# alanqrwang/nwhead

Hardware: AMD Instinct MI355X
Metric: query-predictions/sec (higher is better)
Workload: dtype f32; 1 GPU; K3 predict('full'): B=256 queries/step vs bank N=50000 d=512 C=200, bank sharded 1-way, 26 query batches coalesced per launch; B=256, N_support=50000, d=512, C=200, parallelism=support-shard x1

## Files before the change

nwhead_amd/csrc/fused_f16p.h:

```cpp
#pragma once
#include "fused_impl.h"
#include "persistent_pipe.h"

namespace nw {
namespace {

template <int RS, int QB, bool TWO = false>
struct PCfg : PipeCfg<16 * RS, 64 * QB, NCONS, NLOAD, TWO ? 3 : 4> {};

template <int RS, int KIND, int QB, int NCW = NCONS>
__device__ __forceinline__ void epilogue_p(f32x4 (&acc)[QB][RS], const float* hdr, int nrun, int2 bnd,
                                           const float* __restrict__ logit_scale, float* __restrict__ ws_m,
                                           float* __restrict__ ws_den, float* __restrict__ ws_num, int B, int N,
                                           int q0, int s0, int st, int wave, int lane
#ifdef NW_DIAG_FUSED
                                           , unsigned long long (&diag_)[8], unsigned long long& last_
#endif
                                           ) {
    using P = PCfg<RS, QB>;
    constexpr int BS = P::BS;
    constexpr bool NEED_NORM = (KIND != NW_SCORE_DOT);
    constexpr float L2E = 1.44269504088896340736f;
    typedef float f32x2 __attribute__((ext_vector_type(2)));
    const float* sn2 = hdr;
// ... 83 lines not shown
                    S1[r & 1] = __builtin_fmaf(in1 ? 1.f : 0.f, quad, S1[r & 1]);
                    S2[r & 1] = __builtin_fmaf(in2 ? 1.f : 0.f, quad, S2[r & 1]);
                    if (!(in0 || in1 || in2)) {
#pragma unroll
                        for (int e = 0; e < 4; ++e) {
                            const float c = (float)(16 * r + e), ev = sc[r][e];
                            const float w1 = __builtin_amdgcn_fmed3f(L1 - c, 0.f, 1.f);
                            const float u2 = __builtin_amdgcn_fmed3f(c + M2, 0.f, 1.f);
                            S0[e & 1] = __builtin_fmaf(w1, ev, S0[e & 1]);
                            S2[e & 1] = __builtin_fmaf(u2, ev, S2[e & 1]);
                            S1[e & 1] = __builtin_fmaf((1.f - w1) - u2, ev, S1[e & 1]);
                        }
                    }
                }
            }
            const float s0v = red4(S0[0] + S0[1]);
            float s1v = 0.f, s2v = 0.f;
            if (nrun >= 2) s1v = red4(S1[0] + S1[1]);
            if (nrun == 3) s2v = red4(S2[0] + S2[1]);
            dloc = (s0v + s1v) + s2v;
            if (g == 0 && b < B) {
                ws_num[((size_t)st * BS) * B + b] = s0v;
                if (nrun >= 2) ws_num[((size_t)st * BS + 1) * B + b] = s1v;
                if (nrun == 3) ws_num[((size_t)st * BS + 2) * B + b] = s2v;
            }
        } else {
            float dl[4] = {0.f, 0.f, 0.f, 0.f};
#pragma unroll
            for (int r = 0; r < RS; ++r) dl[r & 3] += (sc[r][0] + sc[r][1]) + (sc[r][2] + sc[r][3]);
            dloc = red4((dl[0] + dl[1]) + (dl[2] + dl[3]));
            for (int run_base = 0; run_base < nrun; run_base += 16) {
                f32x4 Pm = {0.f, 0.f, 0.f, 0.f};
                const int want = run_base + i;
#pragma unroll
                for (int r = 0; r < RS; ++r) {
                    const int4 rid = *reinterpret_cast<const int4*>(runid + 16 * r + 4 * g);
                    Pm = __builtin_amdgcn_mfma_f32_16x16x4f32(rid.x == want ? 1.f : 0.f, sc[r][0], Pm, 0, 0, 0);
                    Pm = __builtin_amdgcn_mfma_f32_16x16x4f32(rid.y == want ? 1.f : 0.f, sc[r][1], Pm, 0, 0, 0);
                    Pm = __builtin_amdgcn_mfma_f32_16x16x4f32(rid.z == want ? 1.f : 0.f, sc[r][2], Pm, 0, 0, 0);
                    Pm = __builtin_amdgcn_mfma_f32_16x16x4f32(rid.w == want ? 1.f : 0.f, sc[r][3], Pm, 0, 0, 0);
                }
                if (b < B) {
#pragma unroll
                    for (int jj = 0; jj < 4; ++jj) {
                        const int run = run_base + 4 * g + jj;
                        if (run < nrun) ws_num[((size_t)st * BS + run) * B + b] = Pm[jj];
                    }
                }
            }
        }
        NW_PSTAMP(4);
        if (g == 0 && b < B) {
            ws_m[(size_t)st * B + b] = mloc;
            ws_den[(size_t)st * B + b] = dloc;
        }
        NW_PSTAMP(5);
    }
}

template <int RS, int KIND, bool TWO, int QB>
__global__ __launch_bounds__(TILE_THREADS, TWO ? 4 : 2) void nw_fused_f16p_kernel(
    const float* __restrict__ q, const float* __restrict__ s, const float* __restrict__ s_norm2,
    const float* __restrict__ s_scale, const float* __restrict__ q_norm2, const float* __restrict__ q_scale,
    const float* __restrict__ logit_scale, const int* __restrict__ ws_runid, const int* __restrict__ ws_nrun, const int* __restrict__ ws_bnd,
    float* __restrict__ ws_m, float* __restrict__ ws_den, float* __restrict__ ws_num, int B, int N, int d,
    int n_stiles, int n_qtiles, int qg) {
    using P = PCfg<RS, QB, TWO>;
    constexpr int BS = P::BS, BQP = P::BQP, TILE_F4 = P::TILE_F4, NB = P::NB;
    constexpr bool SINGLE = TWO || QB > 1;
    static_assert(!(TWO && QB > 1), "two 128-query workgroups do not fit the LDS of a CU");
    static_assert(P::THREADS == TILE_THREADS, "launch bounds");
    static_assert(RS == 8, "the persistent kernel is built for tiles of 128 supports");
    extern __shared__ __attribute__((aligned(16))) char smem[];
    float* hdr0 = reinterpret_cast<float*>(smem);
    float4* stage = reinterpret_cast<float4*>(smem + P::HDR_BYTES);

    const int tid = threadIdx.x, lane = tid & 63;
    const int wave = __builtin_amdgcn_readfirstlane(tid >> 6);
    const int nk = d / BK;
    const PersistentTiles tiles(blockIdx.x, gridDim.x, n_stiles, n_qtiles, qg);
    const int cu = tiles.cu, n_cu = tiles.n_cu, n_local = tiles.n_local;

    if (wave >= P::NCW) {
        persistent_loader<P>(tiles, wave - P::NCW, lane, hdr0, stage, q, s, s_norm2, s_scale, q_norm2, q_scale, ws_runid, B, N,
                             d);
    } else {
        const int i = lane & 15, g = lane >> 4;
        struct Frag {
            float4 bh[QB], bl[QB];
            float4 ah[RS], al[RS];
        };
        const int rsw = (i >> 1) & 7;
        auto load_frags = [&](Frag& f, int buf) {
            const float4* Qs = stage + ((unsigned)buf % NB) * TILE_F4;
            const float4* Ss = Qs + BQP * ROW_F4;
            const int sh = g ^ rsw, sl = (4 + g) ^ rsw;
#pragma unroll
            for (int j = 0; j < QB; ++j) {
                const int qrow = 16 * (QB * wave + j) + i;
                f.bh[j] = Qs[qrow * ROW_F4 + sh];
                f.bl[j] = Qs[qrow * ROW_F4 + sl];
            }
#pragma unroll
            for (int r = 0; r < RS; ++r) {
                f.ah[r] = Ss[(16 * r + i) * ROW_F4 + sh];
                f.al[r] = Ss[(16 * r + i) * ROW_F4 + sl];
            }
        };
        auto mm = [](const float4& a, const float4& b, f32x4 c) {
            return __builtin_amdgcn_mfma_f32_16x16x32_f16(__builtin_bit_cast(half8, a), __builtin_bit_cast(half8, b), c, 0, 0, 0);
        };
        f32x4 acc[QB][RS];
        auto mfma_stage = [&](const Frag& f) {
#pragma unroll
            for (int j = 0; j < QB; ++j)
#pragma unroll
                for (int r = 0; r < RS; ++r) acc[j][r] = mm(f.al[r], f.bh[j], acc[j][r]);
#pragma unroll
            for (int j = 0; j < QB; ++j)
#pragma unroll
                for (int r = 0; r < RS; ++r) acc[j][r] = mm(f.ah[r], f.bl[j], acc[j][r]);
#pragma unroll
            for (int j = 0; j < QB; ++j)
#pragma unroll
                for (int r = 0; r < RS; ++r) acc[j][r] = mm(f.ah[r], f.bh[j], acc[j][r]);
        };
        auto interleave = [&]() {
#pragma unroll
            for (int x = 0; x < 2 * (RS + 1); ++x) {
                __builtin_amdgcn_sched_group_barrier(0x008, 1, 0);
                __builtin_amdgcn_sched_group_barrier(0x100, 1, 0);
            }
            __builtin_amdgcn_sched_group_barrier(0x008, 3 * RS - 2 * (RS + 1), 0);
        };

        tile_barrier();
        int gi = 0;
        int par = 0;
#ifdef NW_DIAG_FUSED
        unsigned long long diag_[8] = {0, 0, 0, 0, 0, 0, 0, 0}, last_ = __builtin_amdgcn_s_memtime();
        const unsigned long long first_ = last_, first_rt_ = __builtin_amdgcn_s_memrealtime();
#endif
        for (int T = cu; T < n_local; T += n_cu) {
            int qt, st;
            tiles.decode(T, qt, st);
            const int q0 = qt * BQP, s0 = st * BS;
            const int nrun = ws_nrun[st];
            const int2 bnd = *reinterpret_cast<const int2*>(ws_bnd + 2 * (size_t)st);

#pragma unroll
            for (int j = 0; j < QB; ++j)
#pragma unroll
                for (int r = 0; r < RS; ++r) acc[j][r] = f32x4{0.f, 0.f, 0.f, 0.f};
            if constexpr (QB > 1) {
                struct F1 { float4 bh[QB]; float4 al[RS]; };
                struct F2 { float4 bl[QB]; float4 ah[RS]; };
                const int sh = g ^ rsw, sl = (4 + g) ^ rsw;
                const int qoff = (16 * QB * wave + i) * ROW_F4, soff = (BQP + i) * ROW_F4;
                auto stage_base = [&](int buf) { return stage + ((unsigned)buf % NB) * TILE_F4; };
                auto rd_bh = [&](const float4* S, int j) { return S[qoff + 16 * j * ROW_F4 + sh]; };
                auto rd_bl = [&](const float4* S, int j) { return S[qoff + 16 * j * ROW_F4 + sl]; };
                auto rd_ah = [&](const float4* S, int r) { return S[soff + 16 * r * ROW_F4 + sh]; };
                auto rd_al = [&](const float4* S, int r) { return S[soff + 16 * r * ROW_F4 + sl]; };
                auto pin = []() { __builtin_amdgcn_sched_barrier(0); };
                auto run_stage = [&](const F1& ac, F1& an, F2& b, int buf_next, auto has_next) {
#ifdef NW_ABL_NORD
                    constexpr bool NXT = false;
// ... 128 lines not shown
```

nwhead_amd/csrc/fused_f16p12.h:

```cpp
#pragma once
#include "fused_f16p.h"

namespace nw {
namespace {

struct P12 : PipeCfg<128, 256, 8, 4, 3> {
    static constexpr int RS = BS / 16, QB = BQP / (16 * NCW);
    static_assert(LDS_BYTES <= 160 * 1024, "LDS of one CU");
};

template <int KIND, bool CAND = false>
__device__ __forceinline__ void epilogue_p12(f32x4 (&acc)[P12::QB][P12::RS], const float* hdr, int nrun, int2 bnd,
                                             float scale, float* __restrict__ ws_m,
                                             float* __restrict__ ws_den, float* __restrict__ ws_num, int B, int N,
                                             int q0, int s0, int st, int wave, int lane, int n_stiles, int k
#ifdef NW_DIAG_FUSED
                                             , unsigned long long (&diag_)[8], unsigned long long& last_
#endif
                                             ) {
    using P = P12;
    constexpr int RS = P::RS, QB = P::QB, BS = P::BS;
    constexpr bool NEED_NORM = (KIND != NW_SCORE_DOT);
    typedef float f32x2 __attribute__((ext_vector_type(2)));
    const float* sn2 = hdr;
    const float* ssc = hdr + P::NH;
    const int* runid = reinterpret_cast<const int*>(hdr + 2 * P::NH);
    const float* qn2 = hdr + 3 * P::NH;
    const float* qsc_s = qn2 + P::BQP;
    const int i = lane & 15, g = lane >> 4;
    using SF = ScoreFactors<KIND>;
    float Cq[QB], Bq[QB];
#pragma unroll
    for (int j = 0; j < QB; ++j) {
        const int qrow = 16 * (QB * wave + j) + i;
        SF::query(NEED_NORM ? qn2[qrow] : 0.f, qsc_s[qrow], scale, Cq[j], Bq[j]);
    }
    NW_PSTAMP(1);
    float sc[QB][RS][4];
#pragma unroll
    for (int r = 0; r < RS; ++r) {
        const float4 n4 = NEED_NORM ? *reinterpret_cast<const float4*>(sn2 + 16 * r + 4 * g) : make_float4(0.f, 0.f, 0.f, 0.f);
        const float4 s4 = *reinterpret_cast<const float4*>(ssc + 16 * r + 4 * g);
        float4 K4, B4;
        SF::support(n4.x, s4.x, K4.x, B4.x);
        SF::support(n4.y, s4.y, K4.y, B4.y);
        SF::support(n4.z, s4.z, K4.z, B4.z);
        SF::support(n4.w, s4.w, K4.w, B4.w);
        float4 B4r = B4;
        asm volatile("" : "+v"(B4r.x), "+v"(B4r.y), "+v"(B4r.z), "+v"(B4r.w));
#pragma unroll
        for (int j = 0; j < QB; ++j) {
            const f32x2 cq = {Cq[j], Cq[j]}, bq = {Bq[j], Bq[j]};
            const float4 Bj = (j == 0) ? B4 : B4r;
            const f32x2 d01 = __builtin_elementwise_fma(f32x2{acc[j][r][0], acc[j][r][1]}, f32x2{K4.x, K4.y} * cq,
                                                        f32x2{Bj.x, Bj.y} + bq);
            const f32x2 d23 = __builtin_elementwise_fma(f32x2{acc[j][r][2], acc[j][r][3]}, f32x2{K4.z, K4.w} * cq,
                                                        f32x2{Bj.z, Bj.w} + bq);
            sc[j][r][0] = SF::finish_abs(d01.x);
            sc[j][r][1] = SF::finish_abs(d01.y);
            sc[j][r][2] = SF::finish_abs(d23.x);
            sc[j][r][3] = SF::finish_abs(d23.y);
            asm volatile("" : "+v"(sc[j][r][0]), "+v"(sc[j][r][1]), "+v"(sc[j][r][2]), "+v"(sc[j][r][3]));
        }
        __builtin_amdgcn_sched_barrier(0);
    }
    NW_PSTAMP(2);
    if constexpr (CAND) {
        int ln = lane;
        asm volatile("" : "+v"(ln));
        const int ci = ln & 15, cg = ln >> 4;
#pragma unroll
        for (int j = 0; j < QB; ++j) {
            float u[RS][4];
#pragma unroll
            for (int r = 0; r < RS; ++r)
#pragma unroll
                for (int e = 0; e < 4; ++e) u[r][e] = SF::DIST ? -sc[j][r][e] : sc[j][r][e];
            tile_candidates<RS>(u, reinterpret_cast<unsigned*>(ws_m), reinterpret_cast<int*>(ws_den), B, N,
                                q0 + 16 * (QB * wave + j) + ci, s0, cg, st, n_stiles, k);
            __builtin_amdgcn_sched_barrier(0);
        }
        return;
    }
    constexpr float WORST = SF::DIST ? INFINITY : -INFINITY;
    if (s0 + BS > N) {
        const int lim = N - s0 - 4 * g;
#pragma unroll
        for (int j = 0; j < QB; ++j)
#pragma unroll
            for (int r = 0; r < RS; ++r)
#pragma unroll
                for (int e = 0; e < 4; ++e)
                    if (16 * r + e >= lim) sc[j][r][e] = WORST;
    }
    auto best = [](float a, float b) { return SF::DIST ? fminf(a, b) : fmaxf(a, b); };
    auto best3 = [&](float a, float b, float c) { return best(best(a, b), c); };
    static_assert(RS == 8, "chain k takes the 16-row blocks k and k + 4");
    float ext[QB];
#pragma unroll
    for (int j = 0; j < QB; ++j) {
        float mx[4];
#pragma unroll
        for (int k = 0; k < 4; ++k) mx[k] = best3(sc[j][k][0], sc[j][k][1], sc[j][k][2]);
#pragma unroll
        for (int k = 0; k < 4; ++k) mx[k] = best3(mx[k], sc[j][k][3], sc[j][k + 4][0]);
#pragma unroll
        for (int k = 0; k < 4; ++k) mx[k] = best3(mx[k], sc[j][k + 4][1], sc[j][k + 4][2]);
#pragma unroll
        for (int k = 0; k < 4; ++k) mx[k] = best(mx[k], sc[j][k + 4][3]);
        ext[j] = best(best3(mx[0], mx[1], mx[2]), mx[3]);
    }
    group4_each(ext, best);
    float mloc[QB], dloc[QB], s0v[QB], s1v[QB] = {0.f, 0.f}, s2v[QB] = {0.f, 0.f};
#pragma unroll
    for (int j = 0; j < QB; ++j) {
        mloc[j] = SF::DIST ? -ext[j] : ext[j];
#pragma unroll
        for (int r = 0; r < RS; ++r)
#pragma unroll
            for (int e = 0; e < 4; ++e)
                sc[j][r][e] = __builtin_amdgcn_exp2f(SF::DIST ? ext[j] - sc[j][r][e] : sc[j][r][e] - ext[j]);
    }
    NW_PSTAMP(3);
    auto add = [](float a, float b) { return a + b; };
    if (nrun <= 3) {
        float S0[QB][2] = {{0.f, 0.f}, {0.f, 0.f}}, S1[QB][2] = {{0.f, 0.f}, {0.f, 0.f}}, S2[QB][2] = {{0.f, 0.f}, {0.f, 0.f}};
        if (nrun == 1) {
#pragma unroll
            for (int r = 0; r < RS; ++r)
#pragma unroll
                for (int j = 0; j < QB; ++j) S0[j][r & 1] += (sc[j][r][0] + sc[j][r][1]) + (sc[j][r][2] + sc[j][r][3]);
        } else {
            const int b1 = bnd.x, b2 = (nrun == 3) ? bnd.y : BS;
            const float L1 = (float)(b1 - 4 * g);
            const float M2 = 1.f - (float)(b2 - 4 * g);
#pragma unroll
            for (int r = 0; r < RS; ++r) {
                const int lo = 16 * r, hi = 16 * r + 16;
                const bool in0 = hi <= b1, in2 = lo >= b2, in1 = lo >= b1 && hi <= b2;
#pragma unroll
                for (int j = 0; j < QB; ++j) {
                    const float quad = (sc[j][r][0] + sc[j][r][1]) + (sc[j][r][2] + sc[j][r][3]);
                    S0[j][r & 1] = __builtin_fmaf(in0 ? 1.f : 0.f, quad, S0[j][r & 1]);
                    S1[j][r & 1] = __builtin_fmaf(in1 ? 1.f : 0.f, quad, S1[j][r & 1]);
                    S2[j][r & 1] = __builtin_fmaf(in2 ? 1.f : 0.f, quad, S2[j][r & 1]);
                }
                if (!(in0 || in1 || in2)) {
#pragma unroll
                    for (int e = 0; e < 4; ++e) {
                        const float c = (float)(16 * r + e);
                        const float w1 = __builtin_amdgcn_fmed3f(L1 - c, 0.f, 1.f);
                        const float u2 = __builtin_amdgcn_fmed3f(c + M2, 0.f, 1.f);
#pragma unroll
                        for (int j = 0; j < QB; ++j) {
                            const float ev = sc[j][r][e];
                            S0[j][e & 1] = __builtin_fmaf(w1, ev, S0[j][e & 1]);
                            S2[j][e & 1] = __builtin_fmaf(u2, ev, S2[j][e & 1]);
                            S1[j][e & 1] = __builtin_fmaf((1.f - w1) - u2, ev, S1[j][e & 1]);
                        }
                    }
                }
            }
        }
        if (nrun == 1) {
            float v[QB] = {S0[0][0] + S0[0][1], S0[1][0] + S0[1][1]};
            group4_each(v, add);
            s0v[0] = v[0], s0v[1] = v[1];
        } else if (nrun == 2) {
            float v[2 * QB] = {S0[0][0] + S0[0][1], S0[1][0] + S0[1][1], S1[0][0] + S1[0][1], S1[1][0] + S1[1][1]};
            group4_each(v, add);
            s0v[0] = v[0], s0v[1] = v[1], s1v[0] = v[2], s1v[1] = v[3];
        } else {
            float v[3 * QB] = {S0[0][0] + S0[0][1], S0[1][0] + S0[1][1], S1[0][0] + S1[0][1],
                               S1[1][0] + S1[1][1], S2[0][0] + S2[0][1], S2[1][0] + S2[1][1]};
            group4_each(v, add);
            s0v[0] = v[0], s0v[1] = v[1], s1v[0] = v[2], s1v[1] = v[3], s2v[0] = v[4], s2v[1] = v[5];
        }
#pragma unroll
        for (int j = 0; j < QB; ++j) dloc[j] = (s0v[j] + s1v[j]) + s2v[j];
    } else {
#pragma unroll
        for (int j = 0; j < QB; ++j) {
            float dl[4] = {0.f, 0.f, 0.f, 0.f};
#pragma unroll
            for (int r = 0; r < RS; ++r) dl[r & 3] += (sc[j][r][0] + sc[j][r][1]) + (sc[j][r][2] + sc[j][r][3]);
            dloc[j] = (dl[0] + dl[1]) + (dl[2] + dl[3]);
        }
        group4_each(dloc, add);
#pragma unroll
        for (int j = 0; j < QB; ++j) {
            const int b = q0 + 16 * (QB * wave + j) + i;
            for (int run_base = 0; run_base < nrun; run_base += 16) {
                f32x4 Pm = {0.f, 0.f, 0.f, 0.f};
                const int want = run_base + i;
#pragma unroll
                for (int r = 0; r < RS; ++r) {
                    const int4 rid = *reinterpret_cast<const int4*>(runid + 16 * r + 4 * g);
                    Pm = __builtin_amdgcn_mfma_f32_16x16x4f32(rid.x == want ? 1.f : 0.f, sc[j][r][0], Pm, 0, 0, 0);
                    Pm = __builtin_amdgcn_mfma_f32_16x16x4f32(rid.y == want ? 1.f : 0.f, sc[j][r][1], Pm, 0, 0, 0);
                    Pm = __builtin_amdgcn_mfma_f32_16x16x4f32(rid.z == want ? 1.f : 0.f, sc[j][r][2], Pm, 0, 0, 0);
                    Pm = __builtin_amdgcn_mfma_f32_16x16x4f32(rid.w == want ? 1.f : 0.f, sc[j][r][3], Pm, 0, 0, 0);
                }
                if (b < B) {
#pragma unroll
                    for (int jj = 0; jj < 4; ++jj) {
                        const int run = run_base + 4 * g + jj;
                        if (run < nrun) ws_num[((size_t)st * BS + run) * B + b] = Pm[jj];
                    }
                }
            }
        }
    }
    NW_PSTAMP(4);
    static_assert(QB == 2, "lane groups 0 / 1 carry query blocks 0 / 1, groups 2 / 3 the same blocks of the next array");
    int ln = lane;
    asm volatile("" : "+v"(ln));
    const int b = q0 + 16 * QB * wave + (ln & 31);
    const bool blk1 = ln & 16, arr1 = ln & 32;
    const size_t tb = (size_t)st * B + b, nb = (size_t)st * BS * B + b;
    if (b < B) {
        const float mv = blk1 ? mloc[1] : mloc[0], dv = blk1 ? dloc[1] : dloc[0];
        (arr1 ? ws_den : ws_m)[tb] = arr1 ? dv : mv;
        if (nrun <= 3) {
            const float n0 = blk1 ? s0v[1] : s0v[0], n1 = blk1 ? s1v[1] : s1v[0], n2 = blk1 ? s2v[1] : s2v[0];
            if (!arr1 || nrun >= 2) ws_num[nb + (arr1 ? B : 0)] = arr1 ? n1 : n0;
            if (!arr1 && nrun == 3) ws_num[nb + 2 * (size_t)B] = n2;
        }
    }
    NW_PSTAMP(5);
}

template <int KIND, bool HALF = false, bool CAND = false>
__global__ __launch_bounds__(P12::THREADS, 3) void nw_fused_f16p_kernel_w12(
    const float* __restrict__ q, const float* __restrict__ s, const float* __restrict__ s_norm2,
    const float* __restrict__ s_scale, const float* __restrict__ q_norm2, const float* __restrict__ q_scale,
    const float* __restrict__ logit_scale, const int* __restrict__ ws_runid, const int* __restrict__ ws_nrun,
    const int* __restrict__ ws_bnd, float* __restrict__ ws_m, float* __restrict__ ws_den, float* __restrict__ ws_num, int B,
    int N, int d, int n_stiles, int n_qtiles, int qg, int k) {
    static_assert(!CAND || HALF, "the candidate form exists for half-precision rows only");
    using P = P12;
    constexpr int RS = P::RS, QB = P::QB, BS = P::BS, BQP = P::BQP, NB = P::NB;
    extern __shared__ __attribute__((aligned(16))) char smem[];
    float* hdr0 = reinterpret_cast<float*>(smem);
    float4* stage = reinterpret_cast<float4*>(smem + P::HDR_BYTES);

    const int tid = threadIdx.x, lane = tid & 63;
    const int wave = __builtin_amdgcn_readfirstlane(tid >> 6);
    const int nk = d / BK;
    const PersistentTiles tiles(blockIdx.x, gridDim.x, n_stiles, n_qtiles, qg);
    const int cu = tiles.cu, n_cu = tiles.n_cu, n_local = tiles.n_local;

    if (wave >= P::NCW) {
        persistent_loader<P, !CAND>(tiles, wave - P::NCW, lane, hdr0, stage, q, s, s_norm2, s_scale, q_norm2, q_scale, ws_runid, B, N,
                             d);
    } else {
        const int i = lane & 15, g = lane >> 4;
        const int rsw = (i >> 1) & 7;
        const int sh = g ^ rsw, sl = (4 + g) ^ rsw;
        const int qoff = (16 * QB * wave + i) * ROW_F4, soff = (BQP + i) * ROW_F4;
        struct QF { float4 bh[QB], bl[QB]; };
        struct SW { float4 al[2], ah[2]; };
        constexpr int NW_ = RS / 2;
#ifdef NW_DIAG_FUSED
        unsigned long long diag_[8] = {0, 0, 0, 0, 0, 0, 0, 0}, last_ = 0;
#endif
#ifdef NW_DIAG_HEAD
        unsigned long long h0_ = 0, h1_ = 0;
#define NW_HEAD_STAMP(t) asm volatile("s_memtime %0" : "=s"(t))
#else
#define NW_HEAD_STAMP(t)
#endif
        auto mm = [](const float4& a, const float4& b, f32x4 c) {
            return __builtin_amdgcn_mfma_f32_16x16x32_f16(__builtin_bit_cast(half8, a), __builtin_bit_cast(half8, b), c, 0, 0, 0);
        };
        auto pin = []() { __builtin_amdgcn_sched_barrier(0); };
        f32x4 acc[QB][RS];
        constexpr int NM = HALF ? 8 : 12;
        auto mm_1 = [&](const SW& w, const QF& f, int p, int m) {
            const int ph = m >> 2, x = (m >> 1) & 1, j = m & 1;
            const float4& a = HALF ? (ph == 0 ? w.ah[x] : w.al[x]) : (ph == 0 ? w.al[x] : w.ah[x]);
            const float4& b = HALF ? (ph == 0 ? f.bh[j] : f.bl[j]) : (ph == 1 ? f.bl[j] : f.bh[j]);
            acc[j][2 * p + x] = mm(a, b, acc[j][2 * p + x]);
        };
        auto mm_w = [&](const SW& w, const QF& f, int p, auto&& behind) {
#pragma unroll
            for (int m = 0; m < NM; ++m) {
                mm_1(w, f, p, m);
                behind(m);
            }
            pin();
        };
        auto nothing = [](int) {};
        typedef const __attribute__((address_space(3))) f32x4 lds_f4;
        const unsigned ring0 = (unsigned)(uintptr_t)(__attribute__((address_space(3))) char*)(char*)stage;
        unsigned a_qh = ring0 + 16u * (qoff + sh), a_ql = ring0 + 16u * (qoff + sl);
        unsigned a_sh = ring0 + 16u * (soff + sh), a_sl = ring0 + 16u * (soff + sl);
        asm volatile("" : "+v"(a_qh), "+v"(a_ql), "+v"(a_sh), "+v"(a_sl));
        auto lds_rd = [](unsigned a, int f4) { return __builtin_bit_cast(float4, *(lds_f4*)(uintptr_t)(a + 16u * f4)); };
        auto q_h = [&](int j) { return lds_rd(a_qh, 16 * j * ROW_F4); };
        auto q_l = [&](int j) { return lds_rd(a_ql, 16 * j * ROW_F4); };
        auto s_h = [&](int blk) { return lds_rd(a_sh, 16 * blk * ROW_F4); };
        auto s_l = [&](int blk) { return lds_rd(a_sl, 16 * blk * ROW_F4); };
        auto advance = [&](int slot, int m) {
            const unsigned step = (slot + 1 == NB) ? 0u - (unsigned)((NB - 1) * P::TILE_F4 * 16) : (unsigned)(P::TILE_F4 * 16);
            unsigned& a = (m == 0) ? a_qh : (m == 1) ? a_ql : (m == 2) ? a_sh : a_sl;
            a += step;
            asm volatile("" : "+v"(a));
        };
        SW wa, wb;
        auto rd_first = [&](QF& f, SW& w, int n) {
            const bool qlo = n >= 4, slo = (n < 4) != HALF;
            const int r = n & 3;
            if (r == 0 || r == 3) {
                const int x = r == 3;
                if (slo) w.al[x] = s_l(x);
                else w.ah[x] = s_h(x);
            } else {
                if (qlo) f.bl[r - 1] = q_l(r - 1);
                else f.bh[r - 1] = q_h(r - 1);
            }
        };
        auto rd_pair = [&](SW& w, int p, int n) {
            const int x = n & 1;
            if ((n < 2) != HALF) w.al[x] = s_l(2 * p + x);
            else w.ah[x] = s_h(2 * p + x);
        };
        auto run_stage = [&](const QF& fp, QF& fc, int slot, auto first) {
            constexpr bool FIRST = decltype(first)::value;
#ifdef NW_ABL_NORD
            constexpr bool RD = FIRST;
#else
            constexpr bool RD = true;
#endif
            if constexpr (FIRST) {
#pragma unroll
                for (int n = 0; n < 8; ++n) {
                    rd_first(fc, wa, n);
                    pin();
                }
            } else {
                NW_HEAD_STAMP(h0_);
                mm_w(wb, fp, NW_ - 1, [&](int m) {
                    if (m == 0) NW_HEAD_STAMP(h1_);
                    if (m < 8) {
                        pin();
                        if (RD) rd_first(fc, wa, m);
                        pin();
                    }
                });
            }
#pragma unroll
            for (int p = 0; p + 1 < NW_; ++p) {
                SW& wr = (p & 1) ? wa : wb;
                mm_w((p & 1) ? wb : wa, fc, p, [&](int m) {
                    if (m < 4) {
                        pin();
                        if (RD) rd_pair(wr, p + 1, m);
                        pin();
                    } else if (p + 2 == NW_ && m < 8) {
                        pin();
                        advance(slot, m - 4);
                        pin();
                    }
                });
            }
            static_assert(NW_ % 2 == 0, "the last pair of a stage sits in wb");
            tile_barrier();
#ifdef NW_DIAG_HEAD
            if (!FIRST) diag_[6] += h1_ - h0_;
#endif
        };
        using Yes = std::integral_constant<bool, true>;
        using No = std::integral_constant<bool, false>;

        float scale = 1.f;
        if (KIND == NW_SCORE_CLIP)
            scale = __builtin_bit_cast(float, __builtin_amdgcn_readfirstlane(__builtin_bit_cast(int, expf(*logit_scale))));
        tile_barrier();
        int gi = 0;
        int par = 0;
        auto next_slot = [&]() {
            const int b = gi;
            gi = (gi + 1 == NB) ? 0 : gi + 1;
            return b;
        };
#ifdef NW_DIAG_FUSED
        last_ = __builtin_amdgcn_s_memtime();
        const unsigned long long first_ = last_, first_rt_ = __builtin_amdgcn_s_memrealtime();
#endif
        for (int T = cu; T < n_local; T += n_cu) {
            int qt, st;
            tiles.decode(T, qt, st);
            const int q0 = qt * BQP, s0 = st * BS;
            int nrun = 0;
            int2 bnd = {0, 0};
            if constexpr (!CAND) {
                nrun = ws_nrun[st];
                bnd = *reinterpret_cast<const int2*>(ws_bnd + 2 * (size_t)st);
            }
#pragma unroll
            for (int j = 0; j < QB; ++j)
#pragma unroll
                for (int r = 0; r < RS; ++r) acc[j][r] = f32x4{0.f, 0.f, 0.f, 0.f};
            QF f0, f1;
#ifdef NW_ABL_NORD
#pragma unroll
            for (int n = 0; n < 8; ++n) rd_first(f1, wa, n);
#endif
            run_stage(f1, f0, next_slot(), Yes{});
            int kt = 1;
            for (; kt + 1 < nk; kt += 2) {
                run_stage(f0, f1, next_slot(), No{});
                run_stage(f1, f0, next_slot(), No{});
            }
            if (kt < nk) {
                run_stage(f0, f1, next_slot(), No{});
                mm_w(wb, f1, NW_ - 1, nothing);
            } else {
                mm_w(wb, f0, NW_ - 1, nothing);
            }
            NW_PSTAMP(0);
#ifndef NW_ABL_NOEPI
            epilogue_p12<KIND, CAND>(acc, hdr0 + par * P::HDR_F, nrun, bnd, scale, ws_m, ws_den, ws_num, B, N, q0, s0, st, wave,
                                     lane, n_stiles, k
#ifdef NW_DIAG_FUSED
                                     , diag_, last_
#endif
                                     );
#else
            keep_acc_alive(acc, ws_m, nrun, bnd);
#endif
            par = (par + 1 == P::NHB) ? 0 : par + 1;
#ifndef NW_DIAG_HEAD
            NW_PSTAMP(6);
#endif
        }
#ifdef NW_DIAG_FUSED
        diag_write_out(diag_, last_, first_, first_rt_);
#endif
    }
}

}
}
```

nwhead_amd/csrc/nw_internal.h:

```cpp
#pragma once
#include <hip/hip_runtime.h>
#include <stdint.h>
#include "../../include/nwhead_hip.h"

#define NW_LOG_EPS 1e-12f
#define NW_NORM_EPS 1e-12f

#define NW_CHECK_LAUNCH()                          \
    do {                                           \
        if (hipGetLastError() != hipSuccess) return NW_ERR_LAUNCH; \
    } while (0)

namespace nw {

int launch_scores(const float* q, const float* s, float* scores, int64_t B, int64_t N, int64_t d,
                  int kind, const float* logit_scale_dev, int sup_batched, hipStream_t st);

int aggregate_slices(int64_t B, int64_t N);
int launch_aggregate(const float* scores, const int64_t* sy, int labels_batched, float* out,
                     float* lse, float* weights, float* m, float* den, float* num, int64_t B,
                     int64_t N, int64_t C, hipStream_t st, float* slice_ws = nullptr, size_t slice_ws_floats = 0);

int launch_merge(const float* m, const float* den, const float* num, float* out, int64_t G,
                 int64_t B, int64_t C, int64_t sm, int64_t sd, int64_t sn, const int64_t* class_lo,
// ... 228 lines not shown
}
__device__ __forceinline__ float group4_min(float x);
__device__ __forceinline__ float group4_max(float x) {
    typedef unsigned u2_ __attribute__((ext_vector_type(2)));
    u2_ r = __builtin_amdgcn_permlane32_swap(__float_as_uint(x), __float_as_uint(x), false, false);
    x = fmaxf(__uint_as_float(r[0]), __uint_as_float(r[1]));
    r = __builtin_amdgcn_permlane16_swap(__float_as_uint(x), __float_as_uint(x), false, false);
    return fmaxf(__uint_as_float(r[0]), __uint_as_float(r[1]));
}

__device__ __forceinline__ float group4_min(float x) {
    typedef unsigned u2_ __attribute__((ext_vector_type(2)));
    u2_ r = __builtin_amdgcn_permlane32_swap(__float_as_uint(x), __float_as_uint(x), false, false);
    x = fminf(__uint_as_float(r[0]), __uint_as_float(r[1]));
    r = __builtin_amdgcn_permlane16_swap(__float_as_uint(x), __float_as_uint(x), false, false);
    return fminf(__uint_as_float(r[0]), __uint_as_float(r[1]));
}

template <int NV, typename Op>
__device__ __forceinline__ void group4_each(float (&v)[NV], Op op) {
    typedef unsigned u2_ __attribute__((ext_vector_type(2)));
    u2_ r[NV];
#pragma unroll
    for (int k = 0; k < NV; ++k) r[k] = __builtin_amdgcn_permlane32_swap(__float_as_uint(v[k]), __float_as_uint(v[k]), false, false);
#pragma unroll
    for (int k = 0; k < NV; ++k) v[k] = op(__uint_as_float(r[k][0]), __uint_as_float(r[k][1]));
#pragma unroll
    for (int k = 0; k < NV; ++k) r[k] = __builtin_amdgcn_permlane16_swap(__float_as_uint(v[k]), __float_as_uint(v[k]), false, false);
#pragma unroll
    for (int k = 0; k < NV; ++k) v[k] = op(__uint_as_float(r[k][0]), __uint_as_float(r[k][1]));
}

__device__ __forceinline__ unsigned group4_max_u32(unsigned x) {
    typedef unsigned u2_ __attribute__((ext_vector_type(2)));
    u2_ r = __builtin_amdgcn_permlane32_swap(x, x, false, false);
    x = max(r[0], r[1]);
    r = __builtin_amdgcn_permlane16_swap(x, x, false, false);
    return max(r[0], r[1]);
}
__device__ __forceinline__ unsigned group4_min_u32(unsigned x) {
    typedef unsigned u2_ __attribute__((ext_vector_type(2)));
    u2_ r = __builtin_amdgcn_permlane32_swap(x, x, false, false);
    x = min(r[0], r[1]);
    r = __builtin_amdgcn_permlane16_swap(x, x, false, false);
    return min(r[0], r[1]);
}

__device__ __forceinline__ unsigned ordered_bits(float f) {
    unsigned b = __float_as_uint(f);
    if ((b & 0x7fffffffu) > 0x7f800000u) return 0xffffffffu;
    if ((b << 1) == 0) b = 0;
    return (b & 0x80000000u) ? ~b : (b | 0x80000000u);
}
__device__ __forceinline__ float ordered_bits_to_float(unsigned u) {
    return __uint_as_float((u & 0x80000000u) ? (u ^ 0x80000000u) : ~u);
}

template <int KIND>
__device__ __forceinline__ float score_from_dot(float dot, float qn2, float sn2, float scale) {
    if (KIND == NW_SCORE_DOT) return dot;
    if (KIND == NW_SCORE_EUCLIDEAN) return -fast_sqrt_pos(qn2 + sn2 - 2.f * dot);
    const float nq = fmaxf(sqrtf(qn2), NW_NORM_EPS), ns = fmaxf(sqrtf(sn2), NW_NORM_EPS);
    const float c = dot / (nq * ns);
    if (KIND == NW_SCORE_COSINE) return c;
    if (KIND == NW_SCORE_CLIP) return scale * c;
    const float a = qn2 / (nq * nq), b = sn2 / (ns * ns);
    return -fast_sqrt_pos(a + b - 2.f * c);
}


template <int KIND>
struct ScoreFactors {
    static constexpr float L2E = 1.44269504088896340736f;
    static constexpr bool DIST = (KIND == NW_SCORE_EUCLIDEAN || KIND == NW_SCORE_HYPERSPHERE);
    static constexpr bool NORMALISED = (KIND == NW_SCORE_HYPERSPHERE || KIND == NW_SCORE_COSINE || KIND == NW_SCORE_CLIP);
    static __device__ __forceinline__ float inv_norm(float n2) {
        return __builtin_amdgcn_rcpf(fmaxf(__builtin_amdgcn_sqrtf(n2), NW_NORM_EPS));
    }
    static __device__ __forceinline__ void support(float n2, float sscale, float& K, float& Base) {
        const float in = NORMALISED ? inv_norm(n2) : 1.f;
        K = sscale * in * (DIST ? -2.f * L2E * L2E : L2E);
        Base = DIST ? (NORMALISED ? n2 * in * in : n2) * (L2E * L2E) : 0.f;
    }
    static __device__ __forceinline__ void query(float n2, float qscale, float clip_scale, float& Cq, float& Bq) {
        const float in = NORMALISED ? inv_norm(n2) : 1.f;
        Cq = qscale * in * (KIND == NW_SCORE_CLIP ? clip_scale : 1.f);
        Bq = DIST ? (NORMALISED ? n2 * in * in : n2) * (L2E * L2E) : 0.f;
    }
    static __device__ __forceinline__ float base_plus(float n2, float Bq, bool separate) {
        if (!DIST) return 0.f;
        const float in = NORMALISED ? inv_norm(n2) : 1.f;
        const float t = NORMALISED ? n2 * in * in : n2;
        return separate ? __fadd_rn(__fmul_rn(t, L2E * L2E), Bq) : __builtin_fmaf(t, L2E * L2E, Bq);
    }
    static __device__ __forceinline__ float finish(float x) { return DIST ? -fast_sqrt_pos(x) : x; }
    static __device__ __forceinline__ float finish_abs(float x) { return DIST ? fast_sqrt_pos(x) : x; }
};

}
```

nwhead_amd/csrc/persistent_pipe.h:

```cpp
#pragma once
#include "tile_core.h"

namespace nw {
namespace {

#ifdef NW_DIAG_FUSED
__device__ unsigned long long nw_diag_p[8 * 1024];
__device__ unsigned long long nw_diag_rt[2 * 1024];
#define NW_PSTAMP(k)                                                                         \
    do {                                                                                     \
        unsigned long long now_;                                                             \
        __builtin_amdgcn_sched_barrier(0);                                                   \
        asm volatile("s_memtime %0\n\ts_waitcnt lgkmcnt(0)" : "=s"(now_)::"memory");         \
        __builtin_amdgcn_sched_barrier(0);                                                   \
        diag_[k] += now_ - last_;                                                            \
        last_ = now_;                                                                        \
    } while (0)

__device__ __forceinline__ void diag_write_out(const unsigned long long (&diag_)[8], unsigned long long last_,
                                               unsigned long long first_, unsigned long long first_rt_) {
    if (threadIdx.x == 0 && blockIdx.x < 1024) {
        for (int k = 0; k < 7; ++k) nw_diag_p[8 * blockIdx.x + k] = diag_[k];
        nw_diag_p[8 * blockIdx.x + 7] = last_ - first_;
        nw_diag_rt[2 * blockIdx.x] = first_rt_;
        nw_diag_rt[2 * blockIdx.x + 1] = __builtin_amdgcn_s_memrealtime();
    }
}
#else
#define NW_PSTAMP(k)
#endif

template <int QB, int RS>
__device__ __forceinline__ void keep_acc_alive(const f32x4 (&acc)[QB][RS], float* ws_m, int nrun, int2 bnd) {
    f32x4 sum_ = {0.f, 0.f, 0.f, 0.f};
    for (int j = 0; j < QB; ++j)
        for (int r = 0; r < RS; ++r) sum_ += acc[j][r];
    if (sum_[0] + sum_[1] + sum_[2] + sum_[3] == 12345.678f) ws_m[threadIdx.x] = sum_[0] + nrun + bnd.x;
}

template <int BS_, int BQP_, int NCW_, int NLW_, int NB_>
struct PipeCfg {
    static constexpr int BS = BS_, BQP = BQP_, NCW = NCW_, NLW = NLW_;
    static constexpr int THREADS = 64 * (NCW + NLW);
    static constexpr int NB = NB_;
    static constexpr int AHEAD = NB - 1;
    static constexpr int TILE_F4 = (BQP + BS) * ROW_F4;
    static constexpr int NT = (BQP + BS) / 8;
    static constexpr int NI = NT / NLW;
    static constexpr int NQI = BQP / 8 / NLW;
    static constexpr int N64 = (BS + 63) / 64;
    static constexpr int NH = N64 * 64;
    static constexpr int HDR_F = 3 * NH + 2 * BQP;
    static constexpr int NP = 3 * N64 + 2 * (BQP / 64);
    static constexpr int HPW = (NP + NLW - 1) / NLW;
    static constexpr int NHB = 3;
    static constexpr size_t HDR_BYTES = (size_t)NHB * HDR_F * 4;
    static constexpr size_t LDS_BYTES = HDR_BYTES + (size_t)NB * TILE_F4 * 16;
    static_assert(NT % NLW == 0, "every loader wave issues the same number of pieces");
    static_assert(BQP % (8 * NLW) == 0, "query and support pieces must not share a loader round");
    static_assert(HDR_BYTES % 16 == 0, "stage buffers must stay 16-byte aligned");
    static_assert(NI + HPW < 64, "vmcnt is a 6-bit field");
};

struct PersistentTiles {
    int xcd, cu, n_cu;
    int n_qtiles, qg;
    int ns_x;
    int n_full;
    int nq_x;
    int n_local;
    int grp_tiles;
    __device__ __forceinline__ PersistentTiles(unsigned block, unsigned grid, int n_stiles, int n_qtiles_, int qg_)
        : xcd(block & 7), cu(block >> 3), n_cu(grid >> 3), n_qtiles(n_qtiles_), qg(qg_) {
        ns_x = n_stiles >> 3;
        n_full = ns_x * n_qtiles;
        const int rem = n_stiles & 7;
        nq_x = (n_qtiles - xcd + 7) >> 3;
        n_local = n_full + rem * nq_x;
        grp_tiles = qg * ns_x;
    }
    __device__ __forceinline__ void decode(int L, int& qt, int& st) const {
        if (L >= n_full) {
            const int r = L - n_full, j = r / nq_x;
            st = 8 * ns_x + j;
            qt = xcd + 8 * (r - j * nq_x);
            return;
        }
        const int gi = L / grp_tiles, r = L - gi * grp_tiles;
        const int g = min(qg, n_qtiles - gi * qg);
        const int stl = r / g;
        qt = gi * qg + (r - stl * g);
        st = stl * 8 + xcd;
    }
};

template <class P, bool RUNID = true>
__device__ __forceinline__ void persistent_loader(const PersistentTiles& tiles, int lw, int lane, float* hdr0, float4* stage,
                                                  const float* __restrict__ q, const float* __restrict__ s,
                                                  const float* __restrict__ s_norm2, const float* __restrict__ s_scale,
                                                  const float* __restrict__ q_norm2, const float* __restrict__ q_scale,
                                                  const int* __restrict__ ws_runid, int B, int N, int d) {
    constexpr int BS = P::BS, BQP = P::BQP, NI = P::NI, NLW = P::NLW;
    const int nk = d / BK;
    const int n_local = tiles.n_local, n_cu = tiles.n_cu;
    unsigned voff[NI];
    int iT = tiles.cu, ikt = 0, irot = 0, ipar = 0;
    int iq0 = 0, is0 = 0, ist = 0;
    int gs = 0;
    auto set_tile = [&](int T) {
        int qt, st;
        tiles.decode(T, qt, st);
        iq0 = qt * BQP;
        is0 = st * BS;
        ist = st;
        irot = st % nk;
#pragma unroll
        for (int m = 0; m < NI; ++m) {
            const int R = 8 * (lw + NLW * m) + (lane >> 3);
            const int lslot = (lane & 7) ^ ((R >> 1) & 7);
            const int rel = (m < P::NQI) ? min(iq0 + R, B - 1) - iq0 : min(is0 + R - BQP, N - 1) - is0;
            voff[m] = ((unsigned)rel * (unsigned)d + lslot * 4) * 4u;
        }
    };
    auto dma4 = [&](const void* src, float* dst) {
        __builtin_amdgcn_global_load_lds((const __attribute__((address_space(1))) void*)src,
                                         (__attribute__((address_space(3))) void*)dst, 4, 0, 0);
    };
    auto issue_header = [&]() {
        float* h = hdr0 + ipar * P::HDR_F;
#pragma unroll
        for (int k = 0; k < P::HPW; ++k) {
            const int pc = min(lw + NLW * k, P::NP - 1);
            if (pc < 3 * P::N64) {
                const int arr = pc / P::N64, c = pc - arr * P::N64;
                const int row = is0 + 64 * c + lane;
                float* dst = h + arr * P::NH + 64 * c;
                if (arr == 0) dma4(s_norm2 + min(row, N - 1), dst);
                else if (arr == 1) dma4(s_scale + min(row, N - 1), dst);
                else if constexpr (RUNID) dma4(ws_runid + (size_t)ist * BS + 64 * c + lane, dst);
                else dma4(s_scale + min(row, N - 1), h + P::NH + 64 * c);
            } else {
                const int qp = pc - 3 * P::N64, arr = qp / (BQP / 64), c = qp - arr * (BQP / 64);
                const int row = min(iq0 + 64 * c + lane, B - 1);
                dma4((arr == 0 ? q_norm2 : q_scale) + row, h + 3 * P::NH + arr * BQP + 64 * c);
            }
        }
    };
    bool young_hdr = false;
    auto issue_next = [&]() {
        if (iT >= n_local) return false;
        int kc = ikt + irot;
        if (kc >= nk) kc -= nk;
        float4* buf = stage + gs * P::TILE_F4;
        const char* qb = reinterpret_cast<const char*>(q + (size_t)iq0 * d) + (size_t)kc * BK * 4;
        const char* sb = reinterpret_cast<const char*>(s + (size_t)is0 * d) + (size_t)kc * BK * 4;
#ifndef NW_ABL_NODMA
#pragma unroll
        for (int m = 0; m < NI; ++m) {
            const char* g = ((m < P::NQI) ? qb : sb) + voff[m];
            __builtin_amdgcn_global_load_lds((const __attribute__((address_space(1))) void*)g,
                                             (__attribute__((address_space(3))) void*)(buf + 64 * (lw + NLW * m)), 16, 0, 0);
        }
#else
        (void)qb; (void)sb; (void)buf;
#endif
        young_hdr = (ikt == 0);
        if (young_hdr) issue_header();
        gs = (gs + 1 == P::NB) ? 0 : gs + 1;
        if (++ikt == nk) {
            ikt = 0;
            ipar = (ipar + 1 == P::NHB) ? 0 : ipar + 1;
            iT += n_cu;
            if (iT < n_local) set_tile(iT);
        }
        return true;
    };
#ifndef NW_ABL_NODMA
    constexpr int YOUNG = NI;
#else
    constexpr int YOUNG = 0;
#endif
    auto wait_landed = [&](bool issued) {
        if (!issued) wait_vmcnt<0>();
        else if (young_hdr) wait_vmcnt<YOUNG + P::HPW>();
        else wait_vmcnt<YOUNG>();
    };
    if (iT < n_local) set_tile(iT);
    bool more = true;
#pragma unroll
    for (int k0 = 0; k0 < P::AHEAD; ++k0) more = issue_next();
    wait_landed(more);
    tile_barrier();
    for (int T = tiles.cu; T < n_local; T += n_cu) {
        for (int kt = 0; kt < nk; ++kt) {
            more = issue_next();
            wait_landed(more);
            tile_barrier();
        }
    }
}

}
}
```

Baseline: 8.108 million query-predictions/s.

## Precompute support factors in loader wave and prefetch next tile's first fragments

A loader wave now computes per-support score factors (K, normalised norm term, base) into a new LDS buffer once per tile, so the consumer epilogue only does FMAs instead of recomputing inverse norms per wave. The first-stage fragment reads for the next tile are hoisted into a late hook inside the epilogue, overlapping them with epilogue work. Tile decoding replaces integer divisions with reciprocal-multiply divmod. This adds static LDS, an extra LDS write/read path, and ordering assumptions between loader and consumers.

```diff
diff --git a/nwhead_amd/csrc/fused_f16p.h b/nwhead_amd/csrc/fused_f16p.h
--- a/nwhead_amd/csrc/fused_f16p.h
+++ b/nwhead_amd/csrc/fused_f16p.h
@@ -189,7 +189,7 @@
     const int cu = tiles.cu, n_cu = tiles.n_cu, n_local = tiles.n_local;
 
     if (wave >= P::NCW) {
-        persistent_loader<P>(tiles, wave - P::NCW, lane, hdr0, stage, q, s, s_norm2, s_scale, q_norm2, q_scale, ws_runid, B, N,
+        persistent_loader<P>(tiles, wave - P::NCW, lane, hdr0, nullptr, stage, q, s, s_norm2, s_scale, q_norm2, q_scale, ws_runid, B, N,
                              d);
     } else {
         const int i = lane & 15, g = lane >> 4;
diff --git a/nwhead_amd/csrc/fused_f16p12.h b/nwhead_amd/csrc/fused_f16p12.h
--- a/nwhead_amd/csrc/fused_f16p12.h
+++ b/nwhead_amd/csrc/fused_f16p12.h
@@ -6,14 +6,16 @@
 
 struct P12 : PipeCfg<128, 256, 8, 4, 3> {
     static constexpr int RS = BS / 16, QB = BQP / (16 * NCW);
-    static_assert(LDS_BYTES <= 160 * 1024, "LDS of one CU");
+    static constexpr int FAC_F = NHB * NH;
+    static_assert(LDS_BYTES + FAC_F * 4 <= 160 * 1024, "LDS of one CU");
 };
 
-template <int KIND, bool CAND = false>
-__device__ __forceinline__ void epilogue_p12(f32x4 (&acc)[P12::QB][P12::RS], const float* hdr, int nrun, int2 bnd,
+template <int KIND, bool CAND = false, class Late>
+__device__ __forceinline__ void epilogue_p12(f32x4 (&acc)[P12::QB][P12::RS], const float* hdr, const float* fac, int nrun, int2 bnd,
                                              float scale, float* __restrict__ ws_m,
                                              float* __restrict__ ws_den, float* __restrict__ ws_num, int B, int N,
-                                             int q0, int s0, int st, int wave, int lane, int n_stiles, int k
+                                             int q0, int s0, int st, int wave, int lane, int n_stiles, int k,
+                                             Late&& late
 #ifdef NW_DIAG_FUSED
                                              , unsigned long long (&diag_)[8], unsigned long long& last_
 #endif
@@ -37,8 +39,43 @@
     }
     NW_PSTAMP(1);
     float sc[QB][RS][4];
+    struct Fac { float4 K, t, P; };
+    auto factors = [&](int r) {
+        const float4 zero = make_float4(0.f, 0.f, 0.f, 0.f);
+        Fac f;
+        f.K = *reinterpret_cast<const float4*>(ssc + 16 * r + 4 * g);
+        f.t = SF::DIST ? *reinterpret_cast<const float4*>(sn2 + 16 * r + 4 * g) : zero;
+        f.P = SF::DIST ? *reinterpret_cast<const float4*>(fac + 16 * r + 4 * g) : zero;
+        return f;
+    };
+    constexpr bool AHEAD = SF::DIST;
+    Fac nxt = {};
+    if constexpr (!CAND && AHEAD) nxt = factors(0);
 #pragma unroll
     for (int r = 0; r < RS; ++r) {
+        if constexpr (!CAND) {
+            constexpr float L2E2 = SF::L2E * SF::L2E;
+            const Fac cur = AHEAD ? nxt : factors(r);
+            if (AHEAD && r + 1 < RS) nxt = factors(r + 1);
+#pragma unroll
+            for (int j = 0; j < QB; ++j) {
+                const f32x2 cq = {Cq[j], Cq[j]}, bq = {Bq[j], Bq[j]}, l2 = {L2E2, L2E2};
+                f32x2 a01 = {0.f, 0.f}, a23 = {0.f, 0.f};
+                if (SF::DIST) {
+                    a01 = (j == 0) ? __builtin_elementwise_fma(f32x2{cur.t.x, cur.t.y}, l2, bq) : f32x2{cur.P.x, cur.P.y} + bq;
+                    a23 = (j == 0) ? __builtin_elementwise_fma(f32x2{cur.t.z, cur.t.w}, l2, bq) : f32x2{cur.P.z, cur.P.w} + bq;
+                }
+                const f32x2 d01 = __builtin_elementwise_fma(f32x2{acc[j][r][0], acc[j][r][1]}, f32x2{cur.K.x, cur.K.y} * cq, a01);
+                const f32x2 d23 = __builtin_elementwise_fma(f32x2{acc[j][r][2], acc[j][r][3]}, f32x2{cur.K.z, cur.K.w} * cq, a23);
+                sc[j][r][0] = SF::finish_abs(d01.x);
+                sc[j][r][1] = SF::finish_abs(d01.y);
+                sc[j][r][2] = SF::finish_abs(d23.x);
+                sc[j][r][3] = SF::finish_abs(d23.y);
+                asm volatile("" : "+v"(sc[j][r][0]), "+v"(sc[j][r][1]), "+v"(sc[j][r][2]), "+v"(sc[j][r][3]));
+            }
+            __builtin_amdgcn_sched_barrier(0);
+            continue;
+        }
         const float4 n4 = NEED_NORM ? *reinterpret_cast<const float4*>(sn2 + 16 * r + 4 * g) : make_float4(0.f, 0.f, 0.f, 0.f);
         const float4 s4 = *reinterpret_cast<const float4*>(ssc + 16 * r + 4 * g);
         float4 K4, B4;
@@ -80,6 +117,7 @@
                                 q0 + 16 * (QB * wave + j) + ci, s0, cg, st, n_stiles, k);
             __builtin_amdgcn_sched_barrier(0);
         }
+        late();
         return;
     }
     constexpr float WORST = SF::DIST ? INFINITY : -INFINITY;
@@ -213,6 +251,7 @@
     }
     NW_PSTAMP(4);
     static_assert(QB == 2, "lane groups 0 / 1 carry query blocks 0 / 1, groups 2 / 3 the same blocks of the next array");
+    late();
     int ln = lane;
     asm volatile("" : "+v"(ln));
     const int b = q0 + 16 * QB * wave + (ln & 31);
@@ -241,6 +280,7 @@
     using P = P12;
     constexpr int RS = P::RS, QB = P::QB, BS = P::BS, BQP = P::BQP, NB = P::NB;
     extern __shared__ __attribute__((aligned(16))) char smem[];
+    __shared__ __attribute__((aligned(16))) float fac0[P12::FAC_F];
     float* hdr0 = reinterpret_cast<float*>(smem);
     float4* stage = reinterpret_cast<float4*>(smem + P::HDR_BYTES);
 
@@ -251,7 +291,7 @@
     const int cu = tiles.cu, n_cu = tiles.n_cu, n_local = tiles.n_local;
 
     if (wave >= P::NCW) {
-        persistent_loader<P, !CAND>(tiles, wave - P::NCW, lane, hdr0, stage, q, s, s_norm2, s_scale, q_norm2, q_scale, ws_runid, B, N,
+        persistent_loader<P, !CAND, CAND ? -1 : KIND>(tiles, wave - P::NCW, lane, hdr0, fac0, stage, q, s, s_norm2, s_scale, q_norm2, q_scale, ws_runid, B, N,
                              d);
     } else {
         const int i = lane & 15, g = lane >> 4;
@@ -325,6 +365,12 @@
             if ((n < 2) != HALF) w.al[x] = s_l(2 * p + x);
             else w.ah[x] = s_h(2 * p + x);
         };
+#ifdef NW_DIAG_TURN
+        unsigned long long t0_ = 0, t1_ = 0;
+#define NW_TURN_STAMP(t) asm volatile("s_memtime %0" : "=s"(t))
+#else
+#define NW_TURN_STAMP(t)
+#endif
         auto run_stage = [&](const QF& fp, QF& fc, int slot, auto first) {
             constexpr bool FIRST = decltype(first)::value;
 #ifdef NW_ABL_NORD
@@ -332,13 +378,7 @@
 #else
             constexpr bool RD = true;
 #endif
-            if constexpr (FIRST) {
-#pragma unroll
-                for (int n = 0; n < 8; ++n) {
-                    rd_first(fc, wa, n);
-                    pin();
-                }
-            } else {
+            if constexpr (!FIRST) {
                 NW_HEAD_STAMP(h0_);
                 mm_w(wb, fp, NW_ - 1, [&](int m) {
                     if (m == 0) NW_HEAD_STAMP(h1_);
@@ -353,6 +393,7 @@
             for (int p = 0; p + 1 < NW_; ++p) {
                 SW& wr = (p & 1) ? wa : wb;
                 mm_w((p & 1) ? wb : wa, fc, p, [&](int m) {
+                    if (FIRST && p == 0 && m == 0) NW_TURN_STAMP(t1_);
                     if (m < 4) {
                         pin();
                         if (RD) rd_pair(wr, p + 1, m);
@@ -369,6 +410,9 @@
 #ifdef NW_DIAG_HEAD
             if (!FIRST) diag_[6] += h1_ - h0_;
 #endif
+#ifdef NW_DIAG_TURN
+            if (FIRST && t0_) diag_[6] += t1_ - t0_;
+#endif
         };
         using Yes = std::integral_constant<bool, true>;
         using No = std::integral_constant<bool, false>;
@@ -388,7 +432,22 @@
         last_ = __builtin_amdgcn_s_memtime();
         const unsigned long long first_ = last_, first_rt_ = __builtin_amdgcn_s_memrealtime();
 #endif
+        QF f0, f1;
+        auto read_ahead = [&]() {
+#pragma unroll
+            for (int n = 0; n < 8; ++n) {
+                rd_first(f0, wa, n);
+                pin();
+            }
+        };
+        if (cu < n_local) read_ahead();
         for (int T = cu; T < n_local; T += n_cu) {
+            const bool more = T + n_cu < n_local;
+            auto late = [&]() {
+                pin();
+                if (more) read_ahead();
+                pin();
+            };
             int qt, st;
             tiles.decode(T, qt, st);
             const int q0 = qt * BQP, s0 = st * BS;
@@ -402,7 +461,6 @@
             for (int j = 0; j < QB; ++j)
 #pragma unroll
                 for (int r = 0; r < RS; ++r) acc[j][r] = f32x4{0.f, 0.f, 0.f, 0.f};
-            QF f0, f1;
 #ifdef NW_ABL_NORD
 #pragma unroll
             for (int n = 0; n < 8; ++n) rd_first(f1, wa, n);
@@ -421,17 +479,21 @@
             }
             NW_PSTAMP(0);
 #ifndef NW_ABL_NOEPI
-            epilogue_p12<KIND, CAND>(acc, hdr0 + par * P::HDR_F, nrun, bnd, scale, ws_m, ws_den, ws_num, B, N, q0, s0, st, wave,
-                                     lane, n_stiles, k
+            epilogue_p12<KIND, CAND>(acc, hdr0 + par * P::HDR_F, fac0 + par * P::NH, nrun, bnd, scale, ws_m, ws_den, ws_num, B, N, q0, s0, st, wave,
+                                     lane, n_stiles, k, late
 #ifdef NW_DIAG_FUSED
                                      , diag_, last_
 #endif
                                      );
 #else
             keep_acc_alive(acc, ws_m, nrun, bnd);
+            late();
 #endif
             par = (par + 1 == P::NHB) ? 0 : par + 1;
-#ifndef NW_DIAG_HEAD
+#ifdef NW_DIAG_TURN
+            asm volatile("s_memtime %0\n\ts_waitcnt lgkmcnt(0)" : "=s"(t0_));
+#endif
+#if !defined(NW_DIAG_HEAD) && !defined(NW_DIAG_TURN)
             NW_PSTAMP(6);
 #endif
         }
diff --git a/nwhead_amd/csrc/nw_internal.h b/nwhead_amd/csrc/nw_internal.h
--- a/nwhead_amd/csrc/nw_internal.h
+++ b/nwhead_amd/csrc/nw_internal.h
@@ -334,6 +334,12 @@
         K = sscale * in * (DIST ? -2.f * L2E * L2E : L2E);
         Base = DIST ? (NORMALISED ? n2 * in * in : n2) * (L2E * L2E) : 0.f;
     }
+    static __device__ __forceinline__ void support_parts(float n2, float sscale, float& K, float& t, float& Bp) {
+        const float in = NORMALISED ? inv_norm(n2) : 1.f;
+        K = __fmul_rn(__fmul_rn(sscale, in), DIST ? -2.f * L2E * L2E : L2E);
+        t = DIST ? (NORMALISED ? __fmul_rn(__fmul_rn(n2, in), in) : n2) : 0.f;
+        Bp = DIST ? __fmul_rn(t, L2E * L2E) : 0.f;
+    }
     static __device__ __forceinline__ void query(float n2, float qscale, float clip_scale, float& Cq, float& Bq) {
         const float in = NORMALISED ? inv_norm(n2) : 1.f;
         Cq = qscale * in * (KIND == NW_SCORE_CLIP ? clip_scale : 1.f);
diff --git a/nwhead_amd/csrc/persistent_pipe.h b/nwhead_amd/csrc/persistent_pipe.h
--- a/nwhead_amd/csrc/persistent_pipe.h
+++ b/nwhead_amd/csrc/persistent_pipe.h
@@ -62,40 +62,61 @@
     static_assert(NI + HPW < 64, "vmcnt is a 6-bit field");
 };
 
+struct TileDiv {
+    unsigned dv, rcp;
+    __device__ __forceinline__ void set(int d) {
+        dv = (unsigned)max(d, 1);
+        rcp = 0xFFFFFFFFu / dv;
+    }
+    static __device__ __forceinline__ void divmod(unsigned n, unsigned dv, unsigned rcp, int& quo, int& rem) {
+        unsigned q = __umulhi(n, rcp), r = n - q * dv;
+        if (r >= dv) ++q, r -= dv;
+        quo = (int)q, rem = (int)r;
+    }
+    __device__ __forceinline__ void divmod(int n, int& quo, int& rem) const { divmod((unsigned)n, dv, rcp, quo, rem); }
+};
+
 struct PersistentTiles {
     int xcd, cu, n_cu;
     int n_qtiles, qg;
     int ns_x;
     int n_full;
-    int nq_x;
     int n_local;
-    int grp_tiles;
+    TileDiv by_nq;
+    TileDiv by_grp;
+    TileDiv by_qg;
+    TileDiv by_last;
     __device__ __forceinline__ PersistentTiles(unsigned block, unsigned grid, int n_stiles, int n_qtiles_, int qg_)
         : xcd(block & 7), cu(block >> 3), n_cu(grid >> 3), n_qtiles(n_qtiles_), qg(qg_) {
         ns_x = n_stiles >> 3;
         n_full = ns_x * n_qtiles;
         const int rem = n_stiles & 7;
-        nq_x = (n_qtiles - xcd + 7) >> 3;
+        const int nq_x = (n_qtiles - xcd + 7) >> 3;
         n_local = n_full + rem * nq_x;
-        grp_tiles = qg * ns_x;
+        by_nq.set(nq_x);
+        by_grp.set(qg * ns_x);
+        by_qg.set(qg);
+        by_last.set(n_qtiles % max(qg, 1));
     }
     __device__ __forceinline__ void decode(int L, int& qt, int& st) const {
         if (L >= n_full) {
-            const int r = L - n_full, j = r / nq_x;
+            int j, r;
+            by_nq.divmod(L - n_full, j, r);
             st = 8 * ns_x + j;
-            qt = xcd + 8 * (r - j * nq_x);
+            qt = xcd + 8 * r;
             return;
         }
-        const int gi = L / grp_tiles, r = L - gi * grp_tiles;
+        int gi, r, stl, qi;
+        by_grp.divmod(L, gi, r);
         const int g = min(qg, n_qtiles - gi * qg);
-        const int stl = r / g;
-        qt = gi * qg + (r - stl * g);
+        TileDiv::divmod((unsigned)r, (unsigned)g, g == qg ? by_qg.rcp : by_last.rcp, stl, qi);
+        qt = gi * qg + qi;
         st = stl * 8 + xcd;
     }
 };
 
-template <class P, bool RUNID = true>
-__device__ __forceinline__ void persistent_loader(const PersistentTiles& tiles, int lw, int lane, float* hdr0, float4* stage,
+template <class P, bool RUNID = true, int FKIND = -1>
+__device__ __forceinline__ void persistent_loader(const PersistentTiles& tiles, int lw, int lane, float* hdr0, float* fac0, float4* stage,
                                                   const float* __restrict__ q, const float* __restrict__ s,
                                                   const float* __restrict__ s_norm2, const float* __restrict__ s_scale,
                                                   const float* __restrict__ q_norm2, const float* __restrict__ q_scale,
@@ -185,6 +206,34 @@
         else if (young_hdr) wait_vmcnt<YOUNG + P::HPW>();
         else wait_vmcnt<YOUNG>();
     };
+    int cpar = 0;
+    auto make_factors = [&]() {
+        if constexpr (FKIND >= 0) {
+            static_assert(P::NH == 128, "two rows per lane of one wave");
+            using SF = ScoreFactors<FKIND>;
+            if (lw == 0) {
+                const unsigned a = (unsigned)(uintptr_t)(__attribute__((address_space(3))) float*)(hdr0 + cpar * P::HDR_F) + 4u * lane;
+                const unsigned af = (unsigned)(uintptr_t)(__attribute__((address_space(3))) float*)(fac0 + cpar * P::NH) + 4u * lane;
+                float n2[2], sc[2];
+                asm volatile("ds_read_b32 %0, %4\n\tds_read_b32 %1, %4 offset:256\n\t"
+                             "ds_read_b32 %2, %4 offset:%5\n\tds_read_b32 %3, %4 offset:%6\n\ts_waitcnt lgkmcnt(0)"
+                             : "=&v"(n2[0]), "=&v"(n2[1]), "=&v"(sc[0]), "=&v"(sc[1])
+                             : "v"(a), "n"(4 * P::NH), "n"(4 * P::NH + 256)
+                             : "memory");
+#pragma unroll
+                for (int h = 0; h < 2; ++h) {
+                    float K, t, Bp;
+                    SF::support_parts(n2[h], sc[h], K, t, Bp);
+                    asm volatile("ds_write_b32 %0, %1 offset:%2" ::"v"(a), "v"(K), "n"(4 * P::NH + 256 * h) : "memory");
+                    if constexpr (SF::DIST) {
+                        if constexpr (SF::NORMALISED) asm volatile("ds_write_b32 %0, %1 offset:%2" ::"v"(a), "v"(t), "n"(256 * h) : "memory");
+                        asm volatile("ds_write_b32 %0, %1 offset:%2" ::"v"(af), "v"(Bp), "n"(256 * h) : "memory");
+                    }
+                }
+            }
+            cpar = (cpar + 1 == P::NHB) ? 0 : cpar + 1;
+        }
+    };
     if (iT < n_local) set_tile(iT);
     bool more = true;
 #pragma unroll
@@ -194,6 +243,7 @@
     for (int T = tiles.cu; T < n_local; T += n_cu) {
         for (int kt = 0; kt < nk; ++kt) {
             more = issue_next();
+            if (kt == 0) make_factors();
             wait_landed(more);
             tile_barrier();
         }
```

New measurement: 8.202 million query-predictions/s, median of 6. 1.01x the previous value.
